# Ichoran/dbce-video-cpp

Hardware: AMD Instinct MI355X
Metric: frames/s + raw-pixel GB/s, 4096x3072 U8 encode+decode round-trip (higher is better)
Workload: dtype u8

## Files before the change

dbde-video-cpp_amd/csrc/dbde_capi.cpp:

```cpp
#include "../../include/dbde_hip.h"

#include <hip/hip_runtime.h>

#include <cstdarg>
#include <cstdio>
#include <cstdlib>
#include <cstring>
#include <string>
#include <vector>

#include "dbde16_kernels.h"
#include "dbde_binned_kernels.h"
#include "dbde_crop_kernels.h"
#include "dbde_hist_kernels.h"
#include "dbde_kernels.h"
#include "dbde_project_kernels.h"
#include "dbde_roi_kernels.h"
#include "dbde_scaled_kernels.h"
#include "dbde_trace_kernels.h"

using namespace dbde;

namespace {

// ... 558 lines not shown

static int run_index(dbde_hip_ctx *ctx, const uint8_t *d_stream, size_t stream_bytes, const uint64_t *d_frame_offsets,
                     int n_frames, dbde_hip_frame_result *d_results, const DecGeom &dg, uint32_t min_bytes,
                     uint32_t split) {
    int rc = grow(ctx, ctx->chunk_off, ctx->chunk_off_n, (size_t)n_frames * (dg.cpf + 1u), sizeof(uint32_t));
    if (rc) return rc;
    rc = grow(ctx, ctx->frame_ok, ctx->frame_ok_n, (size_t)n_frames, sizeof(uint32_t));
    if (rc) return rc;

    IdxParams ip;
    ip.stream = d_stream;
    ip.frame_offsets = d_frame_offsets;
    ip.stream_bytes = stream_bytes;
    ip.chunk_off = ctx->chunk_off;
    ip.frame_ok = ctx->frame_ok;
    ip.results = d_results;
    ip.T = dg.T;
    ip.chunks_per_frame = dg.cpf;
    ip.min_bytes = min_bytes;
    ip.geom = dg;
    ip.split = 1;
    ip.frame_ctr = nullptr;
    ip.frame_flag = nullptr;
    if (split > 1u) {
        const size_t before = ctx->idx_ctr_n;
        rc = grow(ctx, ctx->idx_ctr, ctx->idx_ctr_n, 2 * (size_t)n_frames, sizeof(uint32_t));
        if (rc) return rc;
        if (ctx->idx_ctr_n != before)
            HIP_TRY(ctx, hipMemsetAsync(ctx->idx_ctr, 0, ctx->idx_ctr_n * sizeof(uint32_t), ctx->stream));
        ip.split = split;
        ip.frame_ctr = ctx->idx_ctr;
        ip.frame_flag = ctx->idx_ctr + n_frames;
    }
    span_begin(ctx, 1);
    HIP_TRY(ctx, launch_decode_index(ip, n_frames, ctx->stream));
    span_end(ctx);
    return DBDE_HIP_OK;
}

int dbde_hip_decode_frames(dbde_hip_ctx *ctx, const uint8_t *d_stream, size_t stream_bytes,
                           const uint64_t *d_frame_offsets, int W, int H, int n_frames, uint8_t *d_images,
                           dbde_hip_frame_result *d_results) {
    if (!ctx) return DBDE_HIP_ERR_ARG;
    Geometry g;
    if (!d_stream || !d_frame_offsets || !d_images || n_frames < 0 || !geometry(W, H, g))
        return fail(ctx, DBDE_HIP_ERR_ARG, "decode_frames: bad argument (W=%d H=%d n=%d)", W, H, n_frames);
// ... 1420 lines not shown
    p.sticky = ctx->sticky;
    p.diag = reinterpret_cast<unsigned long long *>(ctx->diag);
    if (!ctx->enc16_grid) ctx->enc16_grid = (uint32_t)(dbde16::encode16_blocks_per_cu() * ctx->n_cu);
    span_begin(ctx, 0);
    HIP_TRY(ctx, hipMemsetAsync(ctx->w16, 0, need, ctx->stream));
    p.force_tickets = (ctx->exp_flags & 1u) ? 1u : 0u;
    HIP_TRY(ctx, dbde16::launch_encode16(p, n_frames, ctx->enc16_grid, ctx->stream));
    span_end(ctx);
    return DBDE_HIP_OK;
}

int dbde16_hip_decode_frames(dbde_hip_ctx *ctx, const uint8_t *d_stream, size_t stream_bytes, const uint64_t *d_frame_offsets,
                             int W, int H, int n_frames, uint16_t *d_images, dbde_hip_frame_result *d_results) {
    if (!ctx) return DBDE_HIP_ERR_ARG;
    Geometry g;
    if (!d_stream || !d_frame_offsets || !d_images || n_frames < 0 || !geometry(W, H, g))
        return fail(ctx, DBDE_HIP_ERR_ARG, "decode16: bad argument (W=%d H=%d n=%d)", W, H, n_frames);
    if (n_frames == 0) return DBDE_HIP_OK;
    const DecGeom dg = dec_geometry(g.w, g.h, false, dbde16::kChunkTiles16);
    if (dg.cpf > kMaxChunksPerFrame) return fail(ctx, DBDE_HIP_ERR_ARG, "decode16: frame too large");
    const uint64_t n_chunks64 = (uint64_t)n_frames * dg.cpf;
    if (n_chunks64 >= (1ull << 31)) return fail(ctx, DBDE_HIP_ERR_ARG, "decode16: too many chunks in one call");
    HIP_TRY(ctx, hipSetDevice(ctx->device));
    int rc = run_index(ctx, d_stream, stream_bytes, d_frame_offsets, n_frames, d_results, dg, 2u, 1u);
    if (rc) return rc;
    dbde16::DecParams16 p;
    p.stream = d_stream;
    p.stream_bytes = stream_bytes;
    p.frame_offsets = d_frame_offsets;
    p.images = d_images;
    p.chunk_off = ctx->chunk_off;
    p.frame_ok = ctx->frame_ok;
    p.frame_pixels = g.pixels;
    p.W = W; p.H = H; p.w = g.w; p.h = g.h; p.T = g.T;
    p.chunks_per_frame = dg.cpf;
    p.diag = reinterpret_cast<unsigned long long *>(ctx->diag);
    span_begin(ctx, 2);
    HIP_TRY(ctx, dbde16::launch_decode16(p, n_frames, ctx->stream));
    span_end(ctx);
    return DBDE_HIP_OK;
}


static bool d2h(dbde_hip_ctx *ctx, void *dst, const void *src, size_t n, uint8_t *via = nullptr) {
    void *land = ctx->host_staging && via ? via : dst;
    if (hipMemcpyAsync(land, src, n, hipMemcpyDeviceToHost, ctx->stream) != hipSuccess ||
        hipStreamSynchronize(ctx->stream) != hipSuccess) return false;
// ... 249 lines not shown
```

dbde-video-cpp_amd/csrc/dbde_kernels.h:

```cpp
#pragma once
#include <hip/hip_runtime.h>
#include <stdint.h>

namespace dbde {

constexpr uint32_t kChunkTiles = 512;
constexpr uint32_t kChunkTilesSmall = 384;

struct DecGeom {
    uint32_t w, h, T;
    uint32_t ct;
    uint32_t pieces;
    uint32_t cpf;
};
__host__ __device__ inline DecGeom dec_geometry(uint32_t w, uint32_t h, bool row_aligned, uint32_t plain_ct = kChunkTiles,
                                                uint32_t cap = kChunkTiles) {
    DecGeom g;
    g.w = w; g.h = h; g.T = w * h;
    if (!row_aligned) {
        g.ct = plain_ct; g.pieces = 1u; g.cpf = (g.T + plain_ct - 1u) / plain_ct;
    } else if (w <= cap) {
        uint32_t rows = cap / w;
        if (rows < 1u) rows = 1u;
        g.ct = rows * w; g.pieces = 1u; g.cpf = (h + rows - 1u) / rows;
// ... 73 lines not shown
    uint32_t w, h, T;
    uint32_t chunks_per_frame, n_chunks;
    uint32_t magic_W;
    unsigned long long *fuse_rec;
    uint32_t fuse_epoch;
    uint32_t fuse_flags;
    DecGeom geom;
    unsigned long long *diag;
};

struct IdxParams {
    const uint8_t *stream;
    const uint64_t *frame_offsets;
    uint64_t stream_bytes;
    uint32_t *chunk_off;
    uint32_t *frame_ok;
    void *results;
    uint32_t T, chunks_per_frame;
    uint32_t min_bytes;
    DecGeom geom;
    uint32_t split;
    uint32_t *frame_ctr;
    uint32_t *frame_flag;
};

struct FrameResultDev {
    uint32_t u64s;
    uint32_t pad_;
    uint64_t index;
    uint64_t elapsed_ns;
    uint64_t consumed;
};

hipError_t launch_encode(const EncParams &p, bool fast_in, bool aligned_out, hipStream_t s);
hipError_t launch_encode16_fast(const EncParams &p, bool fast_in, bool aligned_out, hipStream_t s);
hipError_t launch_encode_small(const EncParams &p, bool fast_in, bool aligned_out, hipStream_t s);
int encode_blocks_per_cu();
hipError_t launch_encode_mid(const EncParams &p, uint32_t n_frames, hipStream_t s);
uint32_t mid_threads_for(uint32_t T, uint32_t max_threads = 1024u);
uint32_t mid_encode_threads_for(uint32_t T);
uint32_t mid_decode_threads_for(uint32_t T);
void decode_mid_blocks_per_cu(int (&per_cu)[2][3]);
hipError_t launch_decode_mid(const struct DecParams &p, uint32_t n_frames, uint32_t n_cu, const int (&per_cu)[2][3], hipStream_t s);
hipError_t launch_encode_frames(const EncParams &p, uint32_t n_frames, hipStream_t s);
uint32_t frames_threads_for(uint32_t T);
hipError_t launch_encode_group(const EncParams &p, uint32_t n_frames, uint32_t n_cu, hipStream_t s);
// ... 28 lines not shown
```

dbde-video-cpp_amd/csrc/dbde_kernels.hip:

```cpp
#include "dbde_kernels.h"

#include "dbde_bits.h"
#include "dbde_device.h"


namespace dbde {

#ifndef DBDE_DIAG_LATE
#define DBDE_DIAG_LATE 34
#endif
#ifdef DBDE_DIAG
#define SF_DECL uint64_t sfd[10] = {0, 0, 0, 0, 0, 0, 0, 0, 0, 0}
#define SF_MARK(i) do { if (threadIdx.x == 0) sfd[i] = wall_clock64(); } while (0)
#define SF_DRAIN() asm volatile("s_waitcnt vmcnt(0) lgkmcnt(0)" ::: "memory")
#define SF_FLUSH(diag, last)                                                                          \
    do {                                                                                              \
        if (threadIdx.x == 0 && (diag)) {                                                             \
            atomicMax(&(diag)[0], ~(unsigned long long)sfd[0]);                                       \
            for (int i_ = 1; i_ < 10; i_++) atomicAdd(&(diag)[i_], (unsigned long long)sfd[i_]);      \
            atomicAdd(&(diag)[10], 1ull);                                                             \
            atomicMax(&(diag)[11], (unsigned long long)sfd[last]);                                    \
            atomicMax(&(diag)[12], (unsigned long long)sfd[0]);                                       \
            atomicAdd(&(diag)[13], (unsigned long long)sfd[0]);                                       \
        }                                                                                             \
    } while (0)
// ... 1348 lines not shown
    return mid_threads_for(T, T <= (unsigned)DBDE_MID_DECODE_MAX_THREADS ? (unsigned)DBDE_MID_DECODE_MAX_THREADS : 1024u);
}

hipError_t launch_encode_mid(const EncParams &p, uint32_t n_frames, hipStream_t s) {
    EncParams q = p;
    q.n_chunks = n_frames;
    q.chunks_per_frame = 1u;
    const uint32_t th = mid_encode_threads_for(p.T), per_wg = th / p.T;
    const dim3 grid((n_frames + per_wg - 1u) / per_wg);
    if (th == 256u) hipLaunchKernelGGL(encode_mid_kernel<256>, grid, dim3(256), 0, s, q);
    else if (th == 512u) hipLaunchKernelGGL(encode_mid_kernel<512>, grid, dim3(512), 0, s, q);
    else hipLaunchKernelGGL(encode_mid_kernel<1024>, grid, dim3(1024), 0, s, q);
    return hipGetLastError();
}

int encode_blocks_per_cu() {
    int n = 0;
    if (hipOccupancyMaxActiveBlocksPerMultiprocessor(&n, encode_kernel<kInFast, true>, kEncThreads, 0) != hipSuccess || n < 1)
        n = 1;
    return n;
}


__global__ __launch_bounds__(1024) void decode_index_kernel(IdxParams p) {
    extern __shared__ __attribute__((aligned(16))) uint32_t s_sum[];
    __shared__ uint32_t s_part[16];
    __shared__ uint32_t s_flags;

    const uint32_t f = blockIdx.x;
    const int tid = threadIdx.x, lane = tid & 63, wave = tid >> 6;
    const uint32_t T = p.T, cpf = p.chunks_per_frame;
    const uint64_t off = p.frame_offsets[f];
    const uint64_t meta_t = (1ull + p.min_bytes) * T;
    const uint64_t need = 32ull + meta_t;
    const bool in_range = in_extent(off, need, p.stream_bytes);
    const uint8_t *fb = p.stream + off;

    for (uint32_t k = tid; k < cpf; k += blockDim.x) s_sum[k] = 0;
    if (tid == 0) s_flags = 0;
    __syncthreads();

    uint32_t bad_depth = 0;
    if (in_range) {
        const uint8_t *darr = fb + 24;
        const uint32_t head = (uint32_t)(reinterpret_cast<uintptr_t>(darr) & 15u);
        const uint8_t *a_lo = darr - head;
        const uint32_t npieces = (head + T + 15u) >> 4;
        const bool incr = p.geom.pieces == 1u && p.geom.ct >= 16u;
        const uint32_t step = 16u * blockDim.x, q_step = incr ? step / p.geom.ct : 0u, r_step = incr ? step - q_step * p.geom.ct : 0u;
        uint32_t k_run = 0, rem_run = 0;
        bool have_run = false;
        for (uint32_t i = tid; i < npieces; i += blockDim.x) {
            uint4 q;
            if (a_lo + 16ull * (i + 1u) <= p.stream + p.stream_bytes) {
                q = *reinterpret_cast<const uint4 *>(a_lo + 16ull * i);
            } else {
                uint32_t wq[4] = {0, 0, 0, 0};
                for (uint32_t b = 0; b < 16u; b++) {
                    const uint8_t *src = a_lo + 16ull * i + b;
                    if (src < p.stream + p.stream_bytes) wq[b >> 2] |= (uint32_t)*src << (8u * (b & 3u));
                }
                q = make_uint4(wq[0], wq[1], wq[2], wq[3]);
            }
            uint32_t wv[4] = {q.x, q.y, q.z, q.w};
            const long long pos0 = 16ll * i - (long long)head;
            const uint32_t lo = pos0 < 0 ? 0u : (uint32_t)pos0;
            const uint32_t hi = pos0 + 16 > (long long)T ? T : (uint32_t)(pos0 + 16);
#pragma unroll
            for (int j = 0; j < 4; j++) {
                const long long pj = pos0 + 4 * j;
                uint32_t mask = 0xFFFFFFFFu;
                if (pj < 0) mask = (pj <= -4) ? 0u : (0xFFFFFFFFu << (8 * (int)(-pj)));
                if (pj + 4 > (long long)T) {
                    const long long keep = (long long)T - pj;
                    mask &= keep <= 0 ? 0u : (keep >= 4 ? 0xFFFFFFFFu : (0xFFFFFFFFu >> (8 * (int)(4 - keep))));
                }
                wv[j] &= mask;
                bad_depth |= depth_bytes_bad(wv[j], p.min_bytes);
            }
            uint32_t k_first, k_last;
            if (incr && pos0 >= 0) {
                if (!have_run) { k_run = lo / p.geom.ct; rem_run = lo - k_run * p.geom.ct; have_run = true; }
                k_first = k_run;
                k_last = rem_run + (hi - 1u - lo) >= p.geom.ct ? k_run + 1u : k_run;
                k_run += q_step; rem_run += r_step;
                if (rem_run >= p.geom.ct) { rem_run -= p.geom.ct; k_run++; }
            } else {
                k_first = dec_chunk_of(p.geom, lo);
                k_last = dec_chunk_of(p.geom, hi - 1u);
            }
            if (k_first == k_last || (incr && pos0 >= 0)) {
                const long long bnd = k_first == k_last ? (long long)T : (long long)(k_first + 1u) * p.geom.ct;
                uint32_t sum_lo = 0, sum_hi = 0;
#pragma unroll
                for (int j = 0; j < 4; j++) {
                    const long long nb = bnd - (pos0 + 4 * j);
                    const uint32_t m = nb >= 4 ? 0xFFFFFFFFu : (nb <= 0 ? 0u : (0xFFFFFFFFu >> (8 * (int)(4 - nb))));
                    sum_lo += __builtin_amdgcn_sad_u8(wv[j] & m, 0u, 0u);
                    sum_hi += __builtin_amdgcn_sad_u8(wv[j] & ~m, 0u, 0u);
                }
                if (sum_lo) atomicAdd(&s_sum[k_first], sum_lo);
                if (sum_hi) atomicAdd(&s_sum[k_first + 1u], sum_hi);
            } else {
                for (uint32_t pos = lo; pos < hi; pos++) {
                    const uint32_t b = (uint32_t)((long long)pos - pos0);
                    const uint32_t v = (wv[b >> 2] >> (8u * (b & 3u))) & 0xFFu;
                    if (v) atomicAdd(&s_sum[dec_chunk_of(p.geom, pos)], v);
                }
            }
        }
    }
    if (bad_depth) atomicOr(&s_flags, 1u);
    __syncthreads();

    const uint32_t seg = (cpf + blockDim.x - 1u) / blockDim.x;
    const uint32_t k0 = (uint32_t)tid * seg;
    uint32_t local = 0;
    for (uint32_t k = k0; k < k0 + seg && k < cpf; k++) local += s_sum[k];
    uint32_t incl = local;
#pragma unroll
    for (int o = 1; o < 64; o <<= 1) {
        uint32_t n = __shfl_up(incl, o, 64);
        if (lane >= o) incl += n;
    }
    if (lane == 63) s_part[wave] = incl;
    __syncthreads();
    uint32_t base = 0, total = 0;
    for (int k = 0; k < (int)(blockDim.x >> 6); k++) {
        const uint32_t v = s_part[k];
        if (k < wave) base += v;
        total += v;
    }
    uint32_t run = base + incl - local;
    uint32_t *co = p.chunk_off + (size_t)f * (cpf + 1u);
    for (uint32_t k = k0; k < k0 + seg && k < cpf; k++) {
        co[k] = run;
        run += s_sum[k];
    }
    if (tid == 0) co[cpf] = total;

    if (tid == 0) {
        bool ok = in_range;
        uint32_t field = 0;
        uint64_t index = 0, elapsed = 0, consumed = 20;
        if (in_extent(off, 20, p.stream_bytes)) {
            field = load_u32_bytes(fb);
            index = load_u64_bytes(fb + 4);
            elapsed = f64_to_u64_x86(__longlong_as_double((long long)load_u64_bytes(fb + 12)));
        }
        if (ok) {
            const int32_t nb = (int32_t)load_u32_bytes(fb + 20);
            const int32_t nm = (int32_t)load_u32_bytes(fb + 24 + T);
            const int32_t n64 = (int32_t)load_u32_bytes(fb + 28 + meta_t);
            ok = nb == (int32_t)T && nm == (int32_t)(T * p.min_bytes) && n64 == (int32_t)total && !(s_flags & 1u);
            if (ok && !in_extent(off, need + 8ull * total, p.stream_bytes)) ok = false;
            if (ok) consumed = need + 8ull * total;
        }
        p.frame_ok[f] = ok ? 1u : 0u;
        if (p.results) {
            FrameResultDev *r = reinterpret_cast<FrameResultDev *>(p.results) + f;
            r->u64s = (field == 2u && ok) ? 2u : 0xFFFFFFFFu;
            r->pad_ = 0;
            r->index = index;
            r->elapsed_ns = elapsed;
            r->consumed = consumed;
        }
    }
}

__global__ __launch_bounds__(256) void decode_index_split_kernel(IdxParams p) {
    __shared__ uint32_t s_part[4];
    __shared__ uint32_t s_last;

    const uint32_t f = blockIdx.x / p.split, piece = blockIdx.x - f * p.split;
    const int tid = threadIdx.x, lane = tid & 63, wave = tid >> 6;
    const uint32_t T = p.T, cpf = p.chunks_per_frame;
    const uint64_t off = p.frame_offsets[f];
    const uint64_t meta_t = (1ull + p.min_bytes) * T;
    const uint64_t need = 32ull + meta_t;
    const bool in_range = in_extent(off, need, p.stream_bytes);
    const uint8_t *fb = p.stream + off;
    uint32_t *co = p.chunk_off + (size_t)f * (cpf + 1u);

    const uint32_t per = (cpf + p.split - 1u) / p.split;
    const uint32_t k_begin = piece * per, k_end = k_begin + per < cpf ? k_begin + per : cpf;
    uint32_t bad = 0;
    for (uint32_t k = k_begin + (uint32_t)wave; k < k_end; k += 4u) {
        uint32_t sum = 0;
        if (in_range) {
            const uint8_t *darr = fb + 24;
            const uint32_t c_lo = dec_chunk_begin(p.geom, k), c_hi = dec_chunk_begin(p.geom, k + 1u);
#pragma unroll
            for (uint32_t j = 0; j < 8u; j += 4u) {
                const uint32_t q = c_lo + (uint32_t)lane * 8u + j;
                if (q < c_hi) {
                    uint32_t x;
                    __builtin_memcpy(&x, darr + q, 4);
                    const uint32_t keep = c_hi - q;
                    if (keep < 4u) x &= 0xFFFFFFFFu >> (8u * (4u - keep));
                    bad |= depth_bytes_bad(x, p.min_bytes);
                    sum += __builtin_amdgcn_sad_u8(x, 0u, 0u);
                }
            }
        }
        const uint32_t tot = wave_scan_incl(sum);
        if (lane == 63) __hip_atomic_store(&co[k], tot, __ATOMIC_RELAXED, __HIP_MEMORY_SCOPE_AGENT);
    }
    if (__any((int)(bad != 0u)) && lane == 0) atomicOr(&p.frame_flag[f], 1u);

    asm volatile("s_waitcnt vmcnt(0)" ::: "memory");
    __syncthreads();
    if (tid == 0) s_last = atomicAdd(&p.frame_ctr[f], 1u) == p.split - 1u ? 1u : 0u;
    __syncthreads();
    if (!s_last) return;

    const uint32_t seg = (cpf + 255u) / 256u;
    const uint32_t k0 = (uint32_t)tid * seg;
    uint32_t local = 0;
    for (uint32_t k = k0; k < k0 + seg && k < cpf; k++)
        local += __hip_atomic_load(&co[k], __ATOMIC_RELAXED, __HIP_MEMORY_SCOPE_AGENT);
    const uint32_t incl = wave_scan_incl(local);
    if (lane == 63) s_part[wave] = incl;
    __syncthreads();
    uint32_t base = 0, total = 0;
#pragma unroll
    for (int k = 0; k < 4; k++) {
        const uint32_t v = s_part[k];
        base += k < wave ? v : 0u;
        total += v;
    }
    uint32_t run = base + incl - local;
    for (uint32_t k = k0; k < k0 + seg && k < cpf; k++) {
        const uint32_t v = __hip_atomic_load(&co[k], __ATOMIC_RELAXED, __HIP_MEMORY_SCOPE_AGENT);
        co[k] = run;
        run += v;
    }
    if (tid == 0) {
        co[cpf] = total;
        const uint32_t flags = __hip_atomic_load(&p.frame_flag[f], __ATOMIC_RELAXED, __HIP_MEMORY_SCOPE_AGENT);
        p.frame_flag[f] = 0;
        p.frame_ctr[f] = 0;
        bool ok = in_range;
        uint32_t field = 0;
        uint64_t index = 0, elapsed = 0, consumed = 20;
        if (in_extent(off, 20, p.stream_bytes)) {
            field = load_u32_bytes(fb);
            index = load_u64_bytes(fb + 4);
            elapsed = f64_to_u64_x86(__longlong_as_double((long long)load_u64_bytes(fb + 12)));
        }
        if (ok) {
            const int32_t nb = (int32_t)load_u32_bytes(fb + 20);
            const int32_t nm = (int32_t)load_u32_bytes(fb + 24 + T);
            const int32_t n64 = (int32_t)load_u32_bytes(fb + 28 + meta_t);
            ok = nb == (int32_t)T && nm == (int32_t)(T * p.min_bytes) && n64 == (int32_t)total && !(flags & 1u);
            if (ok && !in_extent(off, need + 8ull * total, p.stream_bytes)) ok = false;
            if (ok) consumed = need + 8ull * total;
        }
        p.frame_ok[f] = ok ? 1u : 0u;
        if (p.results) {
            FrameResultDev *r = reinterpret_cast<FrameResultDev *>(p.results) + f;
            r->u64s = (field == 2u && ok) ? 2u : 0xFFFFFFFFu;
            r->pad_ = 0;
            r->index = index;
            r->elapsed_ns = elapsed;
            r->consumed = consumed;
        }
    }
}

hipError_t launch_decode_index(const IdxParams &p, int n_frames, hipStream_t s) {
    const size_t lds = (size_t)p.chunks_per_frame * sizeof(uint32_t);
    if (lds > 48 * 1024) {
        hipError_t e = hipFuncSetAttribute(reinterpret_cast<const void *>(decode_index_kernel),
                                           hipFuncAttributeMaxDynamicSharedMemorySize, (int)lds);
        if (e != hipSuccess) return e;
    }
    if (p.split > 1u) {
        hipLaunchKernelGGL(decode_index_split_kernel, dim3((uint32_t)n_frames * p.split), dim3(256), 0, s, p);
        return hipGetLastError();
    }
    const uint32_t pieces = (p.T + 15u) / 16u + 1u;
    uint32_t threads = (pieces + 63u) / 64u * 64u;
    threads = threads < 64u ? 64u : (threads > 1024u ? 1024u : threads);
    hipLaunchKernelGGL(decode_index_kernel, dim3(n_frames), dim3(threads), lds, s, p);
    return hipGetLastError();
}

__device__ __forceinline__ uint32_t swz_byte16(uint32_t A) { return A ^ ((A >> 4) & 0xF0u); }

__device__ __forceinline__ void put_byte1(uint32_t &x, uint32_t sh, uint32_t g) {
    asm("v_lshrrev_b32_sdwa %0, %1, %2 dst_sel:BYTE_1 dst_unused:UNUSED_PRESERVE src0_sel:DWORD src1_sel:DWORD" : "+v"(x) : "v"(sh), "v"(g));
}
__device__ __forceinline__ void put_byte2(uint32_t &x, uint32_t sh, uint32_t g) {
    asm("v_lshrrev_b32_sdwa %0, %1, %2 dst_sel:BYTE_2 dst_unused:UNUSED_PRESERVE src0_sel:DWORD src1_sel:DWORD" : "+v"(x) : "v"(sh), "v"(g));
}
__device__ __forceinline__ void put_byte3(uint32_t &x, uint32_t sh, uint32_t g) {
    asm("v_lshrrev_b32_sdwa %0, %1, %2 dst_sel:BYTE_3 dst_unused:UNUSED_PRESERVE src0_sel:DWORD src1_sel:DWORD" : "+v"(x) : "v"(sh), "v"(g));
}

template <bool SWZ>
__device__ __forceinline__ void unpack_tile_from_lds(const uint8_t *s_img, uint32_t byte_base, uint32_t d,
                                                     uint32_t mn, uint32_t (&v)[16]) {
    const uint32_t mn4 = mn * 0x01010101u;
    const bool d8 = d >= 8u;
    uint32_t a = byte_base;
    const uint32_t md = ((1u << d) - 1u) * 0x01010101u;
    const uint32_t md7 = md & 0x7F7F7F7Fu, mdh = md & 0x80808080u;
    const uint32_t mnlo = mn4 & 0x7F7F7F7Fu, mnhi = mn4 & 0x80808080u;
// ... 1385 lines not shown
```

Baseline: 120,000.

## Rework decode index kernel into wave-per-frame, tiny, and split variants

Replaces the one-block-per-frame decode index kernel with three paths chosen by frame count and size. Very small frames are indexed several per wave, mid-count cases use one wave per frame, and the remaining cases use a templated block kernel whose waves each scan a span and combine results in shared memory. Each lane loads 16-byte pieces and sums them with SAD instructions, so the per-frame chunk-offset prefix sums need fewer barriers and the launch shape matches the workload. The 16-bit decoder now also uses the split index path. This adds considerable code complexity and edge-case handling for unaligned tails.

```diff
diff --git a/dbde-video-cpp_amd/csrc/dbde_capi.cpp b/dbde-video-cpp_amd/csrc/dbde_capi.cpp
--- a/dbde-video-cpp_amd/csrc/dbde_capi.cpp
+++ b/dbde-video-cpp_amd/csrc/dbde_capi.cpp
@@ -604,6 +604,7 @@
     ip.split = 1;
     ip.frame_ctr = nullptr;
     ip.frame_flag = nullptr;
+    ip.n_frames = (uint32_t)n_frames;
     if (split > 1u) {
         const size_t before = ctx->idx_ctr_n;
         rc = grow(ctx, ctx->idx_ctr, ctx->idx_ctr_n, 2 * (size_t)n_frames, sizeof(uint32_t));
@@ -2070,7 +2071,8 @@
     const uint64_t n_chunks64 = (uint64_t)n_frames * dg.cpf;
     if (n_chunks64 >= (1ull << 31)) return fail(ctx, DBDE_HIP_ERR_ARG, "decode16: too many chunks in one call");
     HIP_TRY(ctx, hipSetDevice(ctx->device));
-    int rc = run_index(ctx, d_stream, stream_bytes, d_frame_offsets, n_frames, d_results, dg, 2u, 1u);
+    int rc = run_index(ctx, d_stream, stream_bytes, d_frame_offsets, n_frames, d_results, dg, 2u,
+                       index_split_for(n_frames, dg.cpf));
     if (rc) return rc;
     dbde16::DecParams16 p;
     p.stream = d_stream;
diff --git a/dbde-video-cpp_amd/csrc/dbde_kernels.h b/dbde-video-cpp_amd/csrc/dbde_kernels.h
--- a/dbde-video-cpp_amd/csrc/dbde_kernels.h
+++ b/dbde-video-cpp_amd/csrc/dbde_kernels.h
@@ -119,6 +119,7 @@
     uint32_t split;
     uint32_t *frame_ctr;
     uint32_t *frame_flag;
+    uint32_t n_frames;
 };
 
 struct FrameResultDev {
diff --git a/dbde-video-cpp_amd/csrc/dbde_kernels.hip b/dbde-video-cpp_amd/csrc/dbde_kernels.hip
--- a/dbde-video-cpp_amd/csrc/dbde_kernels.hip
+++ b/dbde-video-cpp_amd/csrc/dbde_kernels.hip
@@ -1,6 +1,8 @@
 #include "dbde_kernels.h"
 
 #include "dbde_bits.h"
+#include <type_traits>
+
 #include "dbde_device.h"
 
 
@@ -1395,191 +1397,327 @@
 }
 
 
-__global__ __launch_bounds__(1024) void decode_index_kernel(IdxParams p) {
-    extern __shared__ __attribute__((aligned(16))) uint32_t s_sum[];
-    __shared__ uint32_t s_part[16];
-    __shared__ uint32_t s_flags;
-
-    const uint32_t f = blockIdx.x;
-    const int tid = threadIdx.x, lane = tid & 63, wave = tid >> 6;
+constexpr int kIdxRows = 4;
+constexpr int kIdxTinyFrames = 4;
+constexpr uint32_t kIdxTinyTiles = 1009;
+
+__device__ __attribute__((aligned(16))) const uint32_t k_idx_zeros[4] = {0u, 0u, 0u, 0u};
+
+struct IdxFrame {
+    uint64_t off;
+    const uint8_t *fb;
+    const uint8_t *a_lo;
+    uint32_t head;
+    bool in_range;
+};
+
+__device__ __forceinline__ IdxFrame idx_frame(const IdxParams &p, uint32_t f) {
+    IdxFrame c;
+    c.off = p.frame_offsets[f];
+    c.in_range = in_extent(c.off, 32ull + (1ull + p.min_bytes) * p.T, p.stream_bytes);
+    c.fb = p.stream + c.off;
+    const uint8_t *darr = c.fb + 24;
+    c.head = (uint32_t)(reinterpret_cast<uintptr_t>(darr) & 15u);
+    c.a_lo = darr - c.head;
+    return c;
+}
+
+__device__ __forceinline__ uint32_t idx_load_header(const IdxParams &p, const IdxFrame &c, int lane) {
+    const uint64_t at = lane < 6 ? 4ull * (uint32_t)lane : (lane == 6 ? 24ull + p.T : 28ull + (1ull + p.min_bytes) * p.T);
+    const bool there = lane < 8 && (lane < 5 ? in_extent(c.off, 20, p.stream_bytes) : c.in_range);
+    const uint8_t *src = there ? c.fb + at : reinterpret_cast<const uint8_t *>(k_idx_zeros);
+    uint32_t v;
+    __builtin_memcpy(&v, src, 4);
+    return v;
+}
+
+__device__ __forceinline__ void idx_finish(const IdxParams &p, uint32_t f, const IdxFrame &c, uint32_t total, uint32_t bad,
+                                           uint32_t hv, int lane) {
+    const uint32_t field = (uint32_t)__builtin_amdgcn_readlane((int)hv, 0);
+    const uint64_t index = (uint32_t)__builtin_amdgcn_readlane((int)hv, 1) | ((uint64_t)(uint32_t)__builtin_amdgcn_readlane((int)hv, 2) << 32);
+    const uint64_t el = (uint32_t)__builtin_amdgcn_readlane((int)hv, 3) | ((uint64_t)(uint32_t)__builtin_amdgcn_readlane((int)hv, 4) << 32);
+    const int32_t nb = __builtin_amdgcn_readlane((int)hv, 5), nm = __builtin_amdgcn_readlane((int)hv, 6);
+    const int32_t n64 = __builtin_amdgcn_readlane((int)hv, 7);
+    if (lane != 0) return;
+    const uint64_t need = 32ull + (1ull + p.min_bytes) * p.T;
+    const uint64_t elapsed = f64_to_u64_x86(__longlong_as_double((long long)el));
+    uint64_t consumed = 20;
+    bool ok = c.in_range;
+    if (ok) {
+        ok = nb == (int32_t)p.T && nm == (int32_t)(p.T * p.min_bytes) && n64 == (int32_t)total && !bad;
+        if (ok && !in_extent(c.off, need + 8ull * total, p.stream_bytes)) ok = false;
+        if (ok) consumed = need + 8ull * total;
+    }
+    p.frame_ok[f] = ok ? 1u : 0u;
+    if (p.results) {
+        FrameResultDev *r = reinterpret_cast<FrameResultDev *>(p.results) + f;
+        r->u64s = (field == 2u && ok) ? 2u : 0xFFFFFFFFu;
+        r->pad_ = 0;
+        r->index = index;
+        r->elapsed_ns = elapsed;
+        r->consumed = consumed;
+    }
+}
+
+__device__ __forceinline__ uint4 idx_load_piece(const IdxFrame &c, uint32_t i, bool full) {
+    const uint8_t *src = full ? c.a_lo + 16ull * i : reinterpret_cast<const uint8_t *>(k_idx_zeros);
+    return *reinterpret_cast<const uint4 *>(src);
+}
+template <int N, class F>
+__device__ __forceinline__ void idx_rows(F f) {
+    if constexpr (N > 0) {
+        idx_rows<N - 1>(f);
+        f(std::integral_constant<int, N - 1>{});
+    }
+}
+__device__ __forceinline__ uint4 idx_load_piece_bytes(const IdxFrame &c, uint32_t i, const uint8_t *end) {
+    uint32_t wq[4] = {0, 0, 0, 0};
+#pragma unroll
+    for (uint32_t b = 0; b < 16u; b++) {
+        const uint8_t *src = c.a_lo + 16ull * i + b;
+        if (src < end) wq[b >> 2] |= (uint32_t)*src << (8u * (b & 3u));
+    }
+    return make_uint4(wq[0], wq[1], wq[2], wq[3]);
+}
+
+__device__ __forceinline__ uint32_t idx_keep(int a, int z) {
+    const uint32_t lo = a <= 0 ? 0xFFFFFFFFu : (a >= 4 ? 0u : (0xFFFFFFFFu << (8 * a)));
+    const uint32_t hi = z >= 4 ? 0xFFFFFFFFu : (z <= 0 ? 0u : (0xFFFFFFFFu >> (8 * (4 - z))));
+    return lo & hi;
+}
+__device__ __forceinline__ void idx_clip(uint4 &q, int a, int z) {
+    q.x &= idx_keep(a, z); q.y &= idx_keep(a - 4, z - 4); q.z &= idx_keep(a - 8, z - 8); q.w &= idx_keep(a - 12, z - 12);
+}
+__device__ __forceinline__ uint32_t idx_sum(const uint4 &q) {
+    return __builtin_amdgcn_sad_u8(q.w, 0u, __builtin_amdgcn_sad_u8(q.z, 0u, __builtin_amdgcn_sad_u8(q.y, 0u, __builtin_amdgcn_sad_u8(q.x, 0u, 0u))));
+}
+__device__ __forceinline__ uint32_t idx_sum_below(uint4 q, int d) {
+    idx_clip(q, 0, d);
+    return idx_sum(q);
+}
+__device__ __forceinline__ uint32_t idx_byte(uint64_t q_lo, uint64_t q_hi, uint32_t b) {
+    return (uint32_t)((b < 8u ? q_lo : q_hi) >> (8u * (b & 7u))) & 0xFFu;
+}
+
+struct IdxRun {
+    uint32_t kq, kr, q_step, r_step, ct;
+    bool fast;
+    __device__ __forceinline__ void init(const DecGeom &g, uint32_t e) {
+        fast = g.pieces == 1u && g.ct >= 16u;
+        ct = g.ct; kq = 0; kr = 17u; q_step = 0; r_step = 0;
+        if (fast) {
+            q_step = 1024u / ct; r_step = 1024u - q_step * ct;
+            kq = (e - 1u) / ct; kr = (e - 1u) - kq * ct + 1u;
+        }
+    }
+    __device__ __forceinline__ void next() {
+        kq += q_step; kr += r_step;
+        if (kr > ct) { kr -= ct; kq++; }
+    }
+};
+
+template <class Emit>
+__device__ __forceinline__ void idx_emit_any(const DecGeom &g, uint4 q, int pos0, uint32_t lo, uint32_t hi,
+                                             uint32_t excl, Emit emit) {
+    const uint64_t q_lo = q.x | ((uint64_t)q.y << 32), q_hi = q.z | ((uint64_t)q.w << 32);
+    uint32_t k = dec_chunk_of(g, lo);
+    if (dec_chunk_begin(g, k) != lo) k++;
+    uint32_t acc = excl, pos = lo;
+    for (; k < g.cpf; k++) {
+        const uint32_t b = dec_chunk_begin(g, k);
+        if (b >= hi) break;
+        for (; pos < b; pos++) acc += idx_byte(q_lo, q_hi, (uint32_t)((int)pos - pos0));
+        emit(k, acc);
+    }
+}
+
+template <int ROWS, class Emit>
+__device__ __forceinline__ void idx_wave_span(const IdxParams &p, const IdxFrame &c, uint32_t pb, uint32_t pe, uint32_t t0,
+                                              uint32_t t1, int lane, uint32_t &total, uint32_t &bad, Emit emit) {
+    const uint8_t *end = p.stream + p.stream_bytes;
+    const uint32_t bad_add = p.min_bytes == 1u ? 0x77777777u : 0x6F6F6F6Fu;
+    const uint32_t bad_hi = p.min_bytes == 1u ? 0xF0F0F0F0u : 0xE0E0E0E0u;
+    IdxRun run;
+    run.init(p.geom, 16u * (pb + (uint32_t)lane + 1u) - c.head);
+    uint32_t carry = 0, orx = 0, ory = 0;
+    for (uint32_t i0 = pb; i0 < pe; i0 += 64u * ROWS) {
+        uint4 q[ROWS];
+        uint32_t ps[ROWS];
+        bool act[ROWS], full[ROWS], clipped[ROWS];
+        idx_rows<ROWS>([&](auto R) {
+            constexpr int r = decltype(R)::value;
+            const uint32_t i = i0 + 64u * r + (uint32_t)lane;
+            act[r] = i < pe;
+            full[r] = act[r] && c.a_lo + 16ull * i + 16ull <= end;
+            q[r] = idx_load_piece(c, i, full[r]);
+        });
+        idx_rows<ROWS>([&](auto R) {
+            constexpr int r = decltype(R)::value;
+            const uint32_t i = i0 + 64u * r + (uint32_t)lane;
+            const int pos0 = (int)(16u * i) - (int)c.head;
+            if (act[r] && !full[r]) q[r] = idx_load_piece_bytes(c, i, end);
+            clipped[r] = pos0 < (int)t0 || pos0 + 16 > (int)t1;
+            if (clipped[r]) idx_clip(q[r], (int)t0 - pos0, (int)t1 - pos0);
+            orx |= q[r].x | q[r].y | q[r].z | q[r].w;
+            ory |= (q[r].x + bad_add) | (q[r].y + bad_add) | (q[r].z + bad_add) | (q[r].w + bad_add);
+            ps[r] = idx_sum(q[r]);
+        });
+        idx_rows<ROWS>([&](auto R) {
+            constexpr int r = decltype(R)::value;
+            const uint32_t i = i0 + 64u * r + (uint32_t)lane;
+            const int pos0 = (int)(16u * i) - (int)c.head;
+            const uint32_t incl = wave_scan_incl(ps[r]);
+            const uint32_t excl = carry + incl - ps[r];
+            carry += (uint32_t)__builtin_amdgcn_readlane((int)incl, 63);
+            if (act[r]) {
+                if (run.fast && !clipped[r]) {
+                    if (run.kr <= 16u) emit(run.kq, excl + idx_sum_below(q[r], 16 - (int)run.kr));
+                } else {
+                    const uint32_t lo = pos0 < (int)t0 ? t0 : (uint32_t)pos0;
+                    const uint32_t hi = pos0 + 16 > (int)t1 ? t1 : (uint32_t)(pos0 + 16);
+                    if (lo < hi) idx_emit_any(p.geom, q[r], pos0, lo, hi, excl, emit);
+                }
+            }
+            run.next();
+        });
+    }
+    total = carry;
+    bad = (orx & bad_hi) | (ory & 0x80808080u);
+}
+
+__global__ __launch_bounds__(256) void decode_index_tiny_kernel(IdxParams p) {
+    const int lane = threadIdx.x & 63;
+    const uint32_t wave = (uint32_t)__builtin_amdgcn_readfirstlane((int)(threadIdx.x >> 6));
+    const uint32_t f0 = (blockIdx.x * 4u + wave) * (uint32_t)kIdxTinyFrames;
+    if (f0 >= p.n_frames) return;
+    const uint8_t *end = p.stream + p.stream_bytes;
     const uint32_t T = p.T, cpf = p.chunks_per_frame;
-    const uint64_t off = p.frame_offsets[f];
-    const uint64_t meta_t = (1ull + p.min_bytes) * T;
-    const uint64_t need = 32ull + meta_t;
-    const bool in_range = in_extent(off, need, p.stream_bytes);
-    const uint8_t *fb = p.stream + off;
-
-    for (uint32_t k = tid; k < cpf; k += blockDim.x) s_sum[k] = 0;
-    if (tid == 0) s_flags = 0;
+    IdxFrame c[kIdxTinyFrames];
+    uint4 q[kIdxTinyFrames];
+    uint32_t hv[kIdxTinyFrames];
+    bool have[kIdxTinyFrames], act[kIdxTinyFrames], full[kIdxTinyFrames];
+    idx_rows<kIdxTinyFrames>([&](auto G) {
+        constexpr int g = decltype(G)::value;
+        have[g] = f0 + g < p.n_frames;
+        c[g] = idx_frame(p, have[g] ? f0 + g : f0);
+    });
+    idx_rows<kIdxTinyFrames>([&](auto G) {
+        constexpr int g = decltype(G)::value;
+        const uint32_t npieces = (c[g].head + T + 15u) >> 4;
+        act[g] = have[g] && c[g].in_range && (uint32_t)lane < npieces;
+        full[g] = act[g] && c[g].a_lo + 16ull * (uint32_t)lane + 16ull <= end;
+        q[g] = idx_load_piece(c[g], (uint32_t)lane, full[g]);
+        hv[g] = idx_load_header(p, c[g], lane);
+    });
+    const uint32_t bad_add = p.min_bytes == 1u ? 0x77777777u : 0x6F6F6F6Fu, bad_hi = p.min_bytes == 1u ? 0xF0F0F0F0u : 0xE0E0E0E0u;
+    idx_rows<kIdxTinyFrames>([&](auto G) {
+        constexpr int g = decltype(G)::value;
+        if (!have[g]) return;
+        const uint32_t f = f0 + g;
+        uint32_t *co = p.chunk_off + (size_t)f * (cpf + 1u);
+        const int pos0 = 16 * lane - (int)c[g].head;
+        if (act[g] && !full[g]) q[g] = idx_load_piece_bytes(c[g], (uint32_t)lane, end);
+        const bool clipped = pos0 < 0 || pos0 + 16 > (int)T;
+        if (clipped) idx_clip(q[g], -pos0, (int)T - pos0);
+        const uint32_t bad = ((q[g].x | q[g].y | q[g].z | q[g].w) & bad_hi) |
+                             (((q[g].x + bad_add) | (q[g].y + bad_add) | (q[g].z + bad_add) | (q[g].w + bad_add)) & 0x80808080u);
+        const uint32_t ps = idx_sum(q[g]);
+        const uint32_t incl = wave_scan_incl(ps);
+        const uint32_t total = (uint32_t)__builtin_amdgcn_readlane((int)incl, 63);
+        if (act[g]) {
+            IdxRun run;
+            run.init(p.geom, (uint32_t)(pos0 + 16));
+            auto emit = [&](uint32_t k, uint32_t v) { if (k < cpf) co[k] = v; };
+            if (run.fast && !clipped) {
+                if (run.kr <= 16u) emit(run.kq, incl - ps + idx_sum_below(q[g], 16 - (int)run.kr));
+            } else {
+                const uint32_t lo = pos0 < 0 ? 0u : (uint32_t)pos0, hi = pos0 + 16 > (int)T ? T : (uint32_t)(pos0 + 16);
+                if (lo < hi) idx_emit_any(p.geom, q[g], pos0, lo, hi, incl - ps, emit);
+            }
+        }
+        if (!c[g].in_range)
+            for (uint32_t k = (uint32_t)lane; k < cpf; k += 64u) co[k] = 0u;
+        if (lane == 0) co[cpf] = total;
+        idx_finish(p, f, c[g], total, __any((int)(bad != 0u)) ? 1u : 0u, hv[g], lane);
+    });
+}
+
+__global__ __launch_bounds__(256) void decode_index_wave_kernel(IdxParams p) {
+    const int lane = threadIdx.x & 63;
+    const uint32_t wave = (uint32_t)__builtin_amdgcn_readfirstlane((int)(threadIdx.x >> 6));
+    const uint32_t f = blockIdx.x * 4u + wave;
+    if (f >= p.n_frames) return;
+    const uint32_t T = p.T, cpf = p.chunks_per_frame;
+    const IdxFrame c = idx_frame(p, f);
+    const uint32_t hv = idx_load_header(p, c, lane);
+    uint32_t *co = p.chunk_off + (size_t)f * (cpf + 1u);
+    uint32_t total = 0, bad = 0;
+    if (c.in_range) {
+        idx_wave_span<kIdxRows>(p, c, 0u, (c.head + T + 15u) >> 4, 0u, T, lane, total, bad,
+                                [&](uint32_t k, uint32_t v) { if (k < cpf) co[k] = v; });
+    } else {
+        for (uint32_t k = (uint32_t)lane; k < cpf; k += 64u) co[k] = 0u;
+    }
+    if (lane == 0) co[cpf] = total;
+    idx_finish(p, f, c, total, __any((int)(bad != 0u)) ? 1u : 0u, hv, lane);
+}
+
+template <int THREADS>
+__global__ __launch_bounds__(THREADS) void decode_index_kernel(IdxParams p) {
+    constexpr int NW = THREADS / 64;
+    extern __shared__ __attribute__((aligned(16))) uint32_t s_off[];
+    __shared__ uint32_t s_tot[NW], s_bad[NW], s_base[NW + 1];
+    __shared__ uint32_t s_any, s_last;
+
+    const uint32_t f = blockIdx.x / p.split, part = blockIdx.x - f * p.split;
+    const int tid = threadIdx.x, lane = tid & 63;
+    const uint32_t wave = (uint32_t)__builtin_amdgcn_readfirstlane(tid >> 6);
+    const uint32_t cpf = p.chunks_per_frame;
+    const IdxFrame c = idx_frame(p, f);
+    uint32_t *co = p.chunk_off + (size_t)f * (cpf + 1u);
+    const uint32_t hv = wave == 0u ? idx_load_header(p, c, lane) : 0u;
+
+    const uint32_t per = (cpf + p.split - 1u) / p.split;
+    const uint32_t k_begin = part * per < cpf ? part * per : cpf, k_end = k_begin + per < cpf ? k_begin + per : cpf;
+    const uint32_t n_k = k_end - k_begin;
+    const uint32_t t0 = dec_chunk_begin(p.geom, k_begin), t1 = dec_chunk_begin(p.geom, k_end);
+    const uint32_t pb = (c.head + t0) >> 4, pe = n_k ? (c.head + t1 + 15u) >> 4 : pb;
+    uint32_t S = ((pe - pb + (uint32_t)NW - 1u) / (uint32_t)NW + 63u) & ~63u;
+    if (S == 0u) S = 64u;
+    uint32_t total_w = 0, bad_w = 0;
+    if (c.in_range) {
+        const uint32_t wb = pb + wave * S < pe ? pb + wave * S : pe, we = wb + S < pe ? wb + S : pe;
+        idx_wave_span<kIdxRows>(p, c, wb, we, t0, t1, lane, total_w, bad_w,
+                                [&](uint32_t k, uint32_t v) { if (k - k_begin < n_k) s_off[k - k_begin] = v; });
+    } else {
+        for (uint32_t j = (uint32_t)tid; j < n_k; j += (uint32_t)THREADS) s_off[j] = 0u;
+    }
+    bad_w = __any((int)(bad_w != 0u)) ? 1u : 0u;
+    if (lane == 0) { s_tot[wave] = total_w; s_bad[wave] = bad_w; }
     __syncthreads();
-
-    uint32_t bad_depth = 0;
-    if (in_range) {
-        const uint8_t *darr = fb + 24;
-        const uint32_t head = (uint32_t)(reinterpret_cast<uintptr_t>(darr) & 15u);
-        const uint8_t *a_lo = darr - head;
-        const uint32_t npieces = (head + T + 15u) >> 4;
-        const bool incr = p.geom.pieces == 1u && p.geom.ct >= 16u;
-        const uint32_t step = 16u * blockDim.x, q_step = incr ? step / p.geom.ct : 0u, r_step = incr ? step - q_step * p.geom.ct : 0u;
-        uint32_t k_run = 0, rem_run = 0;
-        bool have_run = false;
-        for (uint32_t i = tid; i < npieces; i += blockDim.x) {
-            uint4 q;
-            if (a_lo + 16ull * (i + 1u) <= p.stream + p.stream_bytes) {
-                q = *reinterpret_cast<const uint4 *>(a_lo + 16ull * i);
-            } else {
-                uint32_t wq[4] = {0, 0, 0, 0};
-                for (uint32_t b = 0; b < 16u; b++) {
-                    const uint8_t *src = a_lo + 16ull * i + b;
-                    if (src < p.stream + p.stream_bytes) wq[b >> 2] |= (uint32_t)*src << (8u * (b & 3u));
-                }
-                q = make_uint4(wq[0], wq[1], wq[2], wq[3]);
-            }
-            uint32_t wv[4] = {q.x, q.y, q.z, q.w};
-            const long long pos0 = 16ll * i - (long long)head;
-            const uint32_t lo = pos0 < 0 ? 0u : (uint32_t)pos0;
-            const uint32_t hi = pos0 + 16 > (long long)T ? T : (uint32_t)(pos0 + 16);
-#pragma unroll
-            for (int j = 0; j < 4; j++) {
-                const long long pj = pos0 + 4 * j;
-                uint32_t mask = 0xFFFFFFFFu;
-                if (pj < 0) mask = (pj <= -4) ? 0u : (0xFFFFFFFFu << (8 * (int)(-pj)));
-                if (pj + 4 > (long long)T) {
-                    const long long keep = (long long)T - pj;
-                    mask &= keep <= 0 ? 0u : (keep >= 4 ? 0xFFFFFFFFu : (0xFFFFFFFFu >> (8 * (int)(4 - keep))));
-                }
-                wv[j] &= mask;
-                bad_depth |= depth_bytes_bad(wv[j], p.min_bytes);
-            }
-            uint32_t k_first, k_last;
-            if (incr && pos0 >= 0) {
-                if (!have_run) { k_run = lo / p.geom.ct; rem_run = lo - k_run * p.geom.ct; have_run = true; }
-                k_first = k_run;
-                k_last = rem_run + (hi - 1u - lo) >= p.geom.ct ? k_run + 1u : k_run;
-                k_run += q_step; rem_run += r_step;
-                if (rem_run >= p.geom.ct) { rem_run -= p.geom.ct; k_run++; }
-            } else {
-                k_first = dec_chunk_of(p.geom, lo);
-                k_last = dec_chunk_of(p.geom, hi - 1u);
-            }
-            if (k_first == k_last || (incr && pos0 >= 0)) {
-                const long long bnd = k_first == k_last ? (long long)T : (long long)(k_first + 1u) * p.geom.ct;
-                uint32_t sum_lo = 0, sum_hi = 0;
-#pragma unroll
-                for (int j = 0; j < 4; j++) {
-                    const long long nb = bnd - (pos0 + 4 * j);
-                    const uint32_t m = nb >= 4 ? 0xFFFFFFFFu : (nb <= 0 ? 0u : (0xFFFFFFFFu >> (8 * (int)(4 - nb))));
-                    sum_lo += __builtin_amdgcn_sad_u8(wv[j] & m, 0u, 0u);
-                    sum_hi += __builtin_amdgcn_sad_u8(wv[j] & ~m, 0u, 0u);
-                }
-                if (sum_lo) atomicAdd(&s_sum[k_first], sum_lo);
-                if (sum_hi) atomicAdd(&s_sum[k_first + 1u], sum_hi);
-            } else {
-                for (uint32_t pos = lo; pos < hi; pos++) {
-                    const uint32_t b = (uint32_t)((long long)pos - pos0);
-                    const uint32_t v = (wv[b >> 2] >> (8u * (b & 3u))) & 0xFFu;
-                    if (v) atomicAdd(&s_sum[dec_chunk_of(p.geom, pos)], v);
-                }
-            }
-        }
-    }
-    if (bad_depth) atomicOr(&s_flags, 1u);
+    if (tid == 0) {
+        uint32_t run = 0, any = 0;
+        for (int w = 0; w < NW; w++) { s_base[w] = run; run += s_tot[w]; any |= s_bad[w]; }
+        s_base[NW] = run;
+        s_any = any;
+    }
     __syncthreads();
-
-    const uint32_t seg = (cpf + blockDim.x - 1u) / blockDim.x;
-    const uint32_t k0 = (uint32_t)tid * seg;
-    uint32_t local = 0;
-    for (uint32_t k = k0; k < k0 + seg && k < cpf; k++) local += s_sum[k];
-    uint32_t incl = local;
-#pragma unroll
-    for (int o = 1; o < 64; o <<= 1) {
-        uint32_t n = __shfl_up(incl, o, 64);
-        if (lane >= o) incl += n;
-    }
-    if (lane == 63) s_part[wave] = incl;
-    __syncthreads();
-    uint32_t base = 0, total = 0;
-    for (int k = 0; k < (int)(blockDim.x >> 6); k++) {
-        const uint32_t v = s_part[k];
-        if (k < wave) base += v;
-        total += v;
-    }
-    uint32_t run = base + incl - local;
-    uint32_t *co = p.chunk_off + (size_t)f * (cpf + 1u);
-    for (uint32_t k = k0; k < k0 + seg && k < cpf; k++) {
-        co[k] = run;
-        run += s_sum[k];
-    }
-    if (tid == 0) co[cpf] = total;
-
-    if (tid == 0) {
-        bool ok = in_range;
-        uint32_t field = 0;
-        uint64_t index = 0, elapsed = 0, consumed = 20;
-        if (in_extent(off, 20, p.stream_bytes)) {
-            field = load_u32_bytes(fb);
-            index = load_u64_bytes(fb + 4);
-            elapsed = f64_to_u64_x86(__longlong_as_double((long long)load_u64_bytes(fb + 12)));
-        }
-        if (ok) {
-            const int32_t nb = (int32_t)load_u32_bytes(fb + 20);
-            const int32_t nm = (int32_t)load_u32_bytes(fb + 24 + T);
-            const int32_t n64 = (int32_t)load_u32_bytes(fb + 28 + meta_t);
-            ok = nb == (int32_t)T && nm == (int32_t)(T * p.min_bytes) && n64 == (int32_t)total && !(s_flags & 1u);
-            if (ok && !in_extent(off, need + 8ull * total, p.stream_bytes)) ok = false;
-            if (ok) consumed = need + 8ull * total;
-        }
-        p.frame_ok[f] = ok ? 1u : 0u;
-        if (p.results) {
-            FrameResultDev *r = reinterpret_cast<FrameResultDev *>(p.results) + f;
-            r->u64s = (field == 2u && ok) ? 2u : 0xFFFFFFFFu;
-            r->pad_ = 0;
-            r->index = index;
-            r->elapsed_ns = elapsed;
-            r->consumed = consumed;
-        }
-    }
-}
-
-__global__ __launch_bounds__(256) void decode_index_split_kernel(IdxParams p) {
-    __shared__ uint32_t s_part[4];
-    __shared__ uint32_t s_last;
-
-    const uint32_t f = blockIdx.x / p.split, piece = blockIdx.x - f * p.split;
-    const int tid = threadIdx.x, lane = tid & 63, wave = tid >> 6;
-    const uint32_t T = p.T, cpf = p.chunks_per_frame;
-    const uint64_t off = p.frame_offsets[f];
-    const uint64_t meta_t = (1ull + p.min_bytes) * T;
-    const uint64_t need = 32ull + meta_t;
-    const bool in_range = in_extent(off, need, p.stream_bytes);
-    const uint8_t *fb = p.stream + off;
-    uint32_t *co = p.chunk_off + (size_t)f * (cpf + 1u);
-
-    const uint32_t per = (cpf + p.split - 1u) / p.split;
-    const uint32_t k_begin = piece * per, k_end = k_begin + per < cpf ? k_begin + per : cpf;
-    uint32_t bad = 0;
-    for (uint32_t k = k_begin + (uint32_t)wave; k < k_end; k += 4u) {
-        uint32_t sum = 0;
-        if (in_range) {
-            const uint8_t *darr = fb + 24;
-            const uint32_t c_lo = dec_chunk_begin(p.geom, k), c_hi = dec_chunk_begin(p.geom, k + 1u);
-#pragma unroll
-            for (uint32_t j = 0; j < 8u; j += 4u) {
-                const uint32_t q = c_lo + (uint32_t)lane * 8u + j;
-                if (q < c_hi) {
-                    uint32_t x;
-                    __builtin_memcpy(&x, darr + q, 4);
-                    const uint32_t keep = c_hi - q;
-                    if (keep < 4u) x &= 0xFFFFFFFFu >> (8u * (4u - keep));
-                    bad |= depth_bytes_bad(x, p.min_bytes);
-                    sum += __builtin_amdgcn_sad_u8(x, 0u, 0u);
-                }
-            }
-        }
-        const uint32_t tot = wave_scan_incl(sum);
-        if (lane == 63) __hip_atomic_store(&co[k], tot, __ATOMIC_RELAXED, __HIP_MEMORY_SCOPE_AGENT);
-    }
-    if (__any((int)(bad != 0u)) && lane == 0) atomicOr(&p.frame_flag[f], 1u);
+    auto offset_of = [&](uint32_t j) -> uint32_t {
+        if (!c.in_range) return 0u;
+        if (j >= n_k) return s_base[NW];
+        const uint32_t piece = (c.head + dec_chunk_begin(p.geom, k_begin + j)) >> 4;
+        return s_off[j] + s_base[(piece - pb) / S];
+    };
+    if (p.split == 1u) {
+        for (uint32_t j = (uint32_t)tid; j < n_k; j += (uint32_t)THREADS) co[j] = offset_of(j);
+        const uint32_t total = s_base[NW];
+        if (tid == 0) co[cpf] = total;
+        if (wave == 0u) idx_finish(p, f, c, total, s_any, hv, lane);
+        return;
+    }
+    for (uint32_t j = (uint32_t)tid; j < n_k; j += (uint32_t)THREADS)
+        __hip_atomic_store(&co[k_begin + j], offset_of(j + 1u) - offset_of(j), __ATOMIC_RELAXED, __HIP_MEMORY_SCOPE_AGENT);
+    if (s_any && tid == 0) atomicOr(&p.frame_flag[f], 1u);
 
     asm volatile("s_waitcnt vmcnt(0)" ::: "memory");
     __syncthreads();
@@ -1587,19 +1725,19 @@
     __syncthreads();
     if (!s_last) return;
 
-    const uint32_t seg = (cpf + 255u) / 256u;
+    const uint32_t seg = (cpf + (uint32_t)THREADS - 1u) / (uint32_t)THREADS;
     const uint32_t k0 = (uint32_t)tid * seg;
     uint32_t local = 0;
     for (uint32_t k = k0; k < k0 + seg && k < cpf; k++)
         local += __hip_atomic_load(&co[k], __ATOMIC_RELAXED, __HIP_MEMORY_SCOPE_AGENT);
     const uint32_t incl = wave_scan_incl(local);
-    if (lane == 63) s_part[wave] = incl;
+    if (lane == 63) s_tot[wave] = incl;
     __syncthreads();
     uint32_t base = 0, total = 0;
 #pragma unroll
-    for (int k = 0; k < 4; k++) {
-        const uint32_t v = s_part[k];
-        base += k < wave ? v : 0u;
+    for (int k = 0; k < NW; k++) {
+        const uint32_t v = s_tot[k];
+        base += k < (int)wave ? v : 0u;
         total += v;
     }
     uint32_t run = base + incl - local;
@@ -1608,55 +1746,59 @@
         co[k] = run;
         run += v;
     }
-    if (tid == 0) {
-        co[cpf] = total;
-        const uint32_t flags = __hip_atomic_load(&p.frame_flag[f], __ATOMIC_RELAXED, __HIP_MEMORY_SCOPE_AGENT);
-        p.frame_flag[f] = 0;
-        p.frame_ctr[f] = 0;
-        bool ok = in_range;
-        uint32_t field = 0;
-        uint64_t index = 0, elapsed = 0, consumed = 20;
-        if (in_extent(off, 20, p.stream_bytes)) {
-            field = load_u32_bytes(fb);
-            index = load_u64_bytes(fb + 4);
-            elapsed = f64_to_u64_x86(__longlong_as_double((long long)load_u64_bytes(fb + 12)));
-        }
-        if (ok) {
-            const int32_t nb = (int32_t)load_u32_bytes(fb + 20);
-            const int32_t nm = (int32_t)load_u32_bytes(fb + 24 + T);
-            const int32_t n64 = (int32_t)load_u32_bytes(fb + 28 + meta_t);
-            ok = nb == (int32_t)T && nm == (int32_t)(T * p.min_bytes) && n64 == (int32_t)total && !(flags & 1u);
-            if (ok && !in_extent(off, need + 8ull * total, p.stream_bytes)) ok = false;
-            if (ok) consumed = need + 8ull * total;
-        }
-        p.frame_ok[f] = ok ? 1u : 0u;
-        if (p.results) {
-            FrameResultDev *r = reinterpret_cast<FrameResultDev *>(p.results) + f;
-            r->u64s = (field == 2u && ok) ? 2u : 0xFFFFFFFFu;
-            r->pad_ = 0;
-            r->index = index;
-            r->elapsed_ns = elapsed;
-            r->consumed = consumed;
-        }
-    }
-}
-
-hipError_t launch_decode_index(const IdxParams &p, int n_frames, hipStream_t s) {
-    const size_t lds = (size_t)p.chunks_per_frame * sizeof(uint32_t);
+    if (wave == 0u) {
+        uint32_t flags = 0;
+        if (lane == 0) {
+            co[cpf] = total;
+            flags = __hip_atomic_load(&p.frame_flag[f], __ATOMIC_RELAXED, __HIP_MEMORY_SCOPE_AGENT);
+            p.frame_flag[f] = 0;
+            p.frame_ctr[f] = 0;
+        }
+        flags = (uint32_t)__builtin_amdgcn_readfirstlane((int)flags);
+        idx_finish(p, f, c, total, flags & 1u, hv, lane);
+    }
+}
+
+
+static uint32_t index_waves_for(uint32_t n_frames, uint32_t pieces) {
+    uint32_t w = n_frames >= 4096u ? 1u : (n_frames >= 2048u ? 4u : (n_frames >= 1024u ? 8u : 16u));
+    while (w > 1u && pieces < 64u * kIdxRows * w) w = w == 4u ? 1u : w / 2u;
+    return w;
+}
+
+template <int THREADS>
+static hipError_t launch_index_shared(const IdxParams &p, uint32_t grid, size_t lds, hipStream_t s) {
     if (lds > 48 * 1024) {
-        hipError_t e = hipFuncSetAttribute(reinterpret_cast<const void *>(decode_index_kernel),
+        hipError_t e = hipFuncSetAttribute(reinterpret_cast<const void *>(decode_index_kernel<THREADS>),
                                            hipFuncAttributeMaxDynamicSharedMemorySize, (int)lds);
         if (e != hipSuccess) return e;
     }
+    hipLaunchKernelGGL(decode_index_kernel<THREADS>, dim3(grid), dim3(THREADS), lds, s, p);
+    return hipGetLastError();
+}
+
+hipError_t launch_decode_index(const IdxParams &p_in, int n_frames, hipStream_t s) {
+    IdxParams p = p_in;
+    p.n_frames = (uint32_t)n_frames;
+    const uint32_t n = (uint32_t)n_frames, cpf = p.chunks_per_frame;
     if (p.split > 1u) {
-        hipLaunchKernelGGL(decode_index_split_kernel, dim3((uint32_t)n_frames * p.split), dim3(256), 0, s, p);
+        const uint32_t per = (cpf + p.split - 1u) / p.split;
+        return launch_index_shared<256>(p, n * p.split, (size_t)per * sizeof(uint32_t), s);
+    }
+    if (p.T <= kIdxTinyTiles) {
+        const uint32_t per_wg = 4u * (uint32_t)kIdxTinyFrames;
+        hipLaunchKernelGGL(decode_index_tiny_kernel, dim3((n + per_wg - 1u) / per_wg), dim3(256), 0, s, p);
         return hipGetLastError();
     }
-    const uint32_t pieces = (p.T + 15u) / 16u + 1u;
-    uint32_t threads = (pieces + 63u) / 64u * 64u;
-    threads = threads < 64u ? 64u : (threads > 1024u ? 1024u : threads);
-    hipLaunchKernelGGL(decode_index_kernel, dim3(n_frames), dim3(threads), lds, s, p);
-    return hipGetLastError();
+    const uint32_t waves = index_waves_for(n, (p.T + 30u) >> 4);
+    const size_t lds = (size_t)cpf * sizeof(uint32_t);
+    if (waves == 1u) {
+        hipLaunchKernelGGL(decode_index_wave_kernel, dim3((n + 3u) / 4u), dim3(256), 0, s, p);
+        return hipGetLastError();
+    }
+    if (waves == 4u) return launch_index_shared<256>(p, n, lds, s);
+    if (waves == 8u) return launch_index_shared<512>(p, n, lds, s);
+    return launch_index_shared<1024>(p, n, lds, s);
 }
 
 __device__ __forceinline__ uint32_t swz_byte16(uint32_t A) { return A ^ ((A >> 4) & 0xF0u); }
diff --git a/profiles/index_bench.py b/profiles/index_bench.py
--- /dev/null
+++ b/profiles/index_bench.py
@@ -0,0 +1,108 @@
+import argparse
+import json
+import os
+import sys
+
+ROOT = os.path.dirname(os.path.dirname(os.path.abspath(__file__)))
+sys.path.insert(0, ROOT)
+
+COPY_CEILING = 6.29e12
+SEED = 0xDBDE2016
+
+CASES = [
+    ("4096x3072", "frames", 4096, 3072, 1024),
+    ("2048x2048", "frames", 2048, 2048, 1000),
+    ("1921x1081", "frames", 1921, 1081, 2048),
+    ("1921x1081 x6144", "frames", 1921, 1081, 6144),
+    ("1080x1920", "frames", 1080, 1920, 2048),
+    ("1366x768", "frames", 1366, 768, 4096),
+    ("1440x900", "frames", 1440, 900, 2048),
+    ("720x1280", "frames", 720, 1280, 4096),
+    ("320x240", "frames", 320, 240, 16384),
+    ("160x120", "frames", 160, 120, 65536),
+    ("4096x3072 x64", "frames", 4096, 3072, 64),
+    ("4096x3072 x1", "frames", 4096, 3072, 1),
+    ("roi 4096x3072", "roi", 4096, 3072, 1024),
+    ("roi 1921x1081", "roi", 1921, 1081, 2048),
+    ("roi 160x120", "roi", 160, 120, 65536),
+    ("roi 4096x3072 x1", "roi", 4096, 3072, 1),
+    ("dbde16 4096x3072 x128", "frames16", 4096, 3072, 128),
+    ("dbde16 4096x3072 x1", "frames16", 4096, 3072, 1),
+    ("dbde16 1920x1080 x1024", "frames16", 1920, 1080, 1024),
+]
+
+
+def main():
+    ap = argparse.ArgumentParser()
+    ap.add_argument("--steps", type=int, default=20)
+    ap.add_argument("--warmup", type=int, default=3)
+    ap.add_argument("--out", default=None, help="also append the JSON lines to this file")
+    ap.add_argument("--lib", default=None, help="libdbde_hip.so to load instead of the in-tree build")
+    ap.add_argument("--tag", default="", help="label of the library in the JSON lines")
+    ap.add_argument("--only", default=None, help="run the cases whose name contains this")
+    a = ap.parse_args()
+
+    import torch
+    import dbde_video_cpp_amd as dv
+    if a.lib:
+        dv.LIB_PATH = os.path.abspath(a.lib)
+    codec = dv.Codec(0)
+    lines = []
+    for name, kind, W, H, n in CASES:
+        if a.only and a.only not in name:
+            continue
+        T = ((W + 7) // 8) * ((H + 7) // 8)
+        if kind == "frames16":
+            g = torch.Generator(device="cuda").manual_seed(1)
+            imgs = torch.randint(0, 4096, (n, H, W), device="cuda", generator=g, dtype=torch.int32).to(torch.int16)
+            cap = n * int(codec.L.dbde16_hip_max_frame_bytes(W, H))
+            buf = torch.empty(32 + cap + 64, dtype=torch.uint8, device="cuda")
+            offs, sizes = codec.encode_frames16(imgs, W, H, n, buf, 32, cap)
+            out = torch.empty_like(imgs)
+            call = lambda: codec.decode_frames16(buf, 32, total, offs, W, H, n, images=out)
+        else:
+            imgs = codec.synth_frames("mixed", SEED, 0, n, W, H)
+            buf, lead, cap = codec.alloc_stream(W, H, n)
+            offs, sizes = codec.encode_frames(imgs, W, H, n, buf, 32, cap)
+            res = torch.empty((n, 4), dtype=torch.int64, device="cuda")
+            if kind == "frames":
+                out = torch.empty_like(imgs)
+                call = lambda: codec.decode_frames(buf, 32, total, offs, W, H, n, images=out, results=res)
+            else:
+                rw, rh = min(256, W), min(256, H)
+                out = torch.empty((n, rh, rw), dtype=torch.uint8, device="cuda")
+                call = lambda: codec.decode_roi(buf, 32, total, offs, W, H, n, 0, 0, rw, rh, out=out, results=res)
+        codec.sync()
+        total = int((offs[-1] + sizes[-1]).item())
+        for _ in range(a.warmup):
+            call()
+        codec.sync()
+        if kind == "roi":
+            assert torch.equal(out, imgs[:, :rh, :rw]), f"{name}: window differs from the images"
+        else:
+            assert torch.equal(out, imgs), f"{name}: decode differs from the images"
+        codec.timing(True)
+        codec.timing_read(reset=True)
+        for _ in range(a.steps):
+            call()
+        codec.sync()
+        tk = codec.timing_read(reset=True)
+        codec.timing(False)
+        ms, launches = tk["decode_index"][0] / a.steps, tk["decode_index"][1] / a.steps
+        nbytes = n * T
+        lines.append(dict(case=name, decoder=kind, W=W, H=H, frames_per_call=n, lib=a.tag, index_ms=round(ms, 5),
+                          launches=launches, depth_bytes=nbytes,
+                          TBps=round(nbytes / (ms * 1e-3) / 1e12, 3) if ms > 0 else 0.0,
+                          floor_ms=round(nbytes / COPY_CEILING * 1e3, 5),
+                          decode_ms=round(tk["decode"][0] / a.steps, 5)))
+        print(json.dumps(lines[-1]), flush=True)
+        del imgs, buf, out
+    if a.out:
+        with open(a.out, "a") as f:
+            for ln in lines:
+                f.write(json.dumps(ln) + "\n")
+    codec.close()
+
+
+if __name__ == "__main__":
+    main()
```

After: 120,300, median of 6. Within noise of the previous version (+0.3%).
